# r-barnes/richdem

Hardware: NVIDIA H100
Metric: Priority-Flood fill + D8 flow accumulation throughput (higher is better)
Workload: dtype f32

## Files before the change

richdem_b200/csrc/capi.cu:

```cuda
#include "common.cuh"

#include <algorithm>
#include <cstdlib>

namespace rdb {

static thread_local std::string g_last_error;

void capi_set_error(const char *msg) { g_last_error = msg ? msg : "unknown error"; }

Ctx &ctx() {
  static Ctx c;
  return c;
}

static void init_device(int device) {
  Ctx &c = ctx();
  if (c.inited && c.device == device) return;
  if (c.inited) fail("rdb200_init: already initialised on device %d (call rdb200_shutdown first)", c.device);
  int ndev = 0;
  cudaError_t e = cudaGetDeviceCount(&ndev);
  if (e != cudaSuccess || ndev == 0)
    fail("no CUDA device available (%s); librichdem_b200 has no CPU fallback",
         e == cudaSuccess ? "device count is 0" : cudaGetErrorString(e));
// ... 136 lines not shown

}

using namespace rdb;

#define CAPI_TRY try {
#define CAPI_END                    \
  }                                 \
  catch (const std::exception &e) { \
    capi_set_error(e.what());       \
    return 1;                       \
  }                                 \
  catch (...) {                     \
    capi_set_error("unknown C++ exception"); \
    return 1;                       \
  }                                 \
  return 0;

extern "C" {

int rdb200_init(int device) {
  CAPI_TRY
  init_device(device);
  CAPI_END
}

void rdb200_shutdown(void) {
  Ctx &c = ctx();
  if (!c.inited) return;
  cudaSetDevice(c.device);
  cudaStreamSynchronize(c.stream);
  ws_release_all();
  if (c.pinned) cudaFreeHost(c.pinned);
  cudaEventDestroy(c.ev0);
  cudaEventDestroy(c.ev1);
  cudaEventDestroy(c.evk0);
  cudaEventDestroy(c.evk1);
  cudaStreamDestroy(c.own_stream);
  for (int k = 0; k < 2; k++)
    if (c.aux_stream[k]) cudaStreamDestroy(c.aux_stream[k]);
  for (int k = 0; k < 3; k++)
    if (c.aux_event[k]) cudaEventDestroy(c.aux_event[k]);
  const Params keep = c.params;
  c = Ctx();
  c.params = keep;
}

const char *rdb200_last_error(void) { return g_last_error.c_str(); }
int rdb200_version(void) { return RDB200_VERSION; }

int rdb200_set_stream(void *cuda_stream) {
  CAPI_TRY
  ensure_init();
  Ctx &c = ctx();
  RDB_CK(cudaStreamSynchronize(c.stream));
  c.stream = cuda_stream ? (cudaStream_t)cuda_stream : c.own_stream;
  CAPI_END
}

int rdb200_get_stats(rdb200_stats *out) {
  CAPI_TRY
  if (!out) fail("rdb200_get_stats: null pointer");
  *out = ctx().stats;
  CAPI_END
}

int rdb200_set_param(const char *name, int64_t value) {
  CAPI_TRY
  if (!name) fail("rdb200_set_param: null name");
  Params &p = ctx().params;
  const std::string n(name);
  if (n == "reset_defaults") p = Params();
  else if (n == "trim_workspace") {
    if (ctx().inited) {
      RDB_CK(cudaStreamSynchronize(ctx().stream));
      ws_trim();
    }
  }
  else if (n == "fill_max_iters") p.fill_max_iters = value;
  else if (n == "fill_rounds_per_sync") p.fill_rounds_per_sync = value > 0 ? value : 16;
  else if (n == "fill_use_tma") p.fill_use_tma = value;
  else if (n == "fill_external_z") p.fill_external_z = value;
  else if (n == "fill_profile") p.fill_profile = value;
  else if (n == "fill_trace") p.fill_trace = value;
  else if (n == "fill_ordered") p.fill_ordered = value;
  else if (n == "fill_order_rounds") p.fill_order_rounds = value;
  else if (n == "fill_band_rounds") p.fill_band_rounds = value;
  else if (n == "accum_threads") p.accum_threads = value > 0 ? value : 256;
  else if (n == "accum_budget") p.accum_budget = value;
  else if (n == "accum_walk_lanes") p.accum_walk_lanes = value;
  else if (n == "accum_fused_prep") p.accum_fused_prep = value;
  else if (n == "flats_tiled") p.flats_tiled = value;
  else if (n == "flats_pair") p.flats_pair = value;
  else if (n == "flats_fused_classify") p.flats_fused_classify = value;
  else if (n == "fill_multigrid") p.fill_multigrid = value;
  else if (n == "fill_multigrid_min") p.fill_multigrid_min = value;
  else if (n == "fill_vcycle") p.fill_vcycle = value;
  else if (n == "fill_band_multigrid") p.fill_band_multigrid = value;
  else if (n == "flats_uf_tiled") p.flats_uf_tiled = value;
  else if (n == "flowdirs_rolling") p.flowdirs_rolling = value;
  else if (n == "accum_packed") p.accum_packed = value;
  else if (n == "accum_dinf_packed") p.accum_dinf_packed = value;
  else if (n == "accum_dinf_share") p.accum_dinf_share = value;
  else if (n == "flowmet_tarboton_filter") p.flowmet_tarboton_filter = value;
  else if (n == "accum_walk_scan") p.accum_walk_scan = value;
  else if (n == "accum_walk_ahead") p.accum_walk_ahead = value;
  else if (n == "accum_dinf_stats") p.accum_dinf_stats = value;
  else if (n == "accum_dinf_wait") p.accum_dinf_wait = value;
  else fail("rdb200_set_param: unknown parameter '%s'", name);
  CAPI_END
}


int rdb200_fill_depressions_d8_f32(float *dem, int32_t w, int32_t h) {
  CAPI_TRY
  if (!dem) fail("fill_depressions: null dem");
  check_dims(w, h);
  CallScope cs((int64_t)w * h);
  const size_t n = (size_t)w * h;
  DevBuf<float> d(n);
  h2d(d.p, dem, n);
  fill_depressions_dev(d.p, w, h);
  d2h(dem, d.p, n);
  cs.done();
  CAPI_END
}

int rdb200_fill_depressions_d4_f32(float *dem, int32_t w, int32_t h) {
  CAPI_TRY
  if (!dem) fail("fill_depressions: null dem");
  check_dims(w, h);
  CallScope cs((int64_t)w * h);
  const size_t n = (size_t)w * h;
  DevBuf<float> d(n);
  h2d(d.p, dem, n);
  fill_depressions_dev(d.p, w, h, true);
  d2h(dem, d.p, n);
  cs.done();
  CAPI_END
}

static int pit_mask_host(const float *dem, uint8_t *mask, int32_t w, int32_t h, float nodata, bool topo4) {
  CAPI_TRY
  if (!dem || !mask) fail("pit_mask: null pointer");
  check_dims(w, h);
  CallScope cs((int64_t)w * h);
  const size_t n = (size_t)w * h;
  DevBuf<float> d(n);
  DevBuf<uint8_t> m(n);
  h2d(d.p, dem, n);
  pit_mask_dev(d.p, m.p, w, h, nodata, topo4);
  d2h(mask, m.p, n);
  cs.done();
  CAPI_END
}
int rdb200_pit_mask_d8_f32(const float *dem, uint8_t *mask, int32_t w, int32_t h, float nodata) {
  return pit_mask_host(dem, mask, w, h, nodata, false);
}
int rdb200_pit_mask_d4_f32(const float *dem, uint8_t *mask, int32_t w, int32_t h, float nodata) {
  return pit_mask_host(dem, mask, w, h, nodata, true);
}

static int has_depressions_host(const float *dem, int32_t w, int32_t h, int32_t *out, bool topo4) {
  CAPI_TRY
  if (!dem || !out) fail("has_depressions: null pointer");
  check_dims(w, h);
// ... 707 lines not shown
```

richdem_b200/csrc/common.cuh:

```cuda
#pragma once

#include <cuda.h>
#include <cuda_runtime.h>

#include <cstdarg>
#include <cstdint>
#include <cstdio>
#include <cstring>
#include <stdexcept>
#include <string>
#include <vector>

#include "../../include/richdem_b200.h"

struct rdb200_fill_state;

namespace rdb {

struct Error : std::runtime_error {
  using std::runtime_error::runtime_error;
};

[[noreturn]] inline void fail(const char *fmt, ...) {
  char buf[1024];
  va_list ap;
  va_start(ap, fmt);
  vsnprintf(buf, sizeof(buf), fmt, ap);
  va_end(ap);
  throw Error(buf);
}

#define RDB_CK(expr)                                                                        \
  do {                                                                                      \
    cudaError_t _e = (expr);                                                                \
    if (_e != cudaSuccess)                                                                  \
      ::rdb::fail("%s failed at %s:%d: %s", #expr, __FILE__, __LINE__, cudaGetErrorString(_e)); \
  } while (0)

__host__ __device__ __forceinline__ int d8dx(int n) {
  return (int)((0x6a41u >> (2 * n)) & 3u) - 1;
}
__host__ __device__ __forceinline__ int d8dy(int n) {
  return (int)((0x2a405u >> (2 * n)) & 3u) - 1;
}

struct Params {
  int64_t fill_max_iters = 0;
  int64_t fill_rounds_per_sync = 16;
  int64_t fill_use_tma = 1;
  int64_t fill_external_z = 1;
  int64_t fill_ordered = 1;
  int64_t fill_order_rounds = 0;
  int64_t fill_band_rounds = 0;
  int64_t fill_profile = 0;
  int64_t fill_trace = 0;
  int64_t fill_multigrid = 8;
  int64_t fill_vcycle = 8;
  int64_t fill_band_multigrid = 0;
  int64_t fill_multigrid_min = 0;
  int64_t flowdirs_rolling = 1;
  int64_t flats_uf_tiled = 1;
  int64_t flats_fused_classify = 1;
  int64_t flats_pair = 1;
  int64_t flats_tiled = 1;
  int64_t accum_dinf_packed = 1;
  int64_t flowmet_tarboton_filter = 1;
  int64_t accum_walk_ahead = 0;
  int64_t accum_walk_scan = 0;
  int64_t accum_dinf_stats = 0;
  int64_t accum_dinf_share = -1;
  int64_t accum_dinf_wait = 0;
  int64_t accum_packed = 1;
  int64_t accum_fused_prep = 1;
  int64_t accum_walk_lanes = 1;
  int64_t accum_threads = 256;
  int64_t accum_budget = 0;
};

struct WsBlock {
  void *ptr;
  size_t bytes;
  bool in_use;
};

struct Ctx {
  bool inited = false;
  int device = -1;
  int num_sms = 0;
  cudaStream_t stream = nullptr;
  cudaStream_t own_stream = nullptr;
  cudaEvent_t ev0 = nullptr, ev1 = nullptr, evk0 = nullptr, evk1 = nullptr;
  cudaStream_t aux_stream[2] = {nullptr, nullptr};
  cudaEvent_t aux_event[3] = {nullptr, nullptr, nullptr};
  std::vector<WsBlock> ws;
  void *pinned = nullptr;
  size_t pinned_bytes = 0;
  rdb200_stats stats;
  Params params;
};

Ctx &ctx();
void ensure_init();
void *ws_alloc(size_t bytes);
void ws_free(void *p);
void ws_release_all();

template <class T>
struct DevBuf {
  T *p = nullptr;
  size_t n = 0;
  DevBuf() = default;
  explicit DevBuf(size_t count) { alloc(count); }
  void alloc(size_t count) {
    reset();
    n = count;
    p = (T *)ws_alloc((count ? count : 1) * sizeof(T));
  }
  void reset() {
    if (p) ws_free(p);
    p = nullptr;
    n = 0;
  }
  ~DevBuf() { reset(); }
  DevBuf(const DevBuf &) = delete;
  DevBuf &operator=(const DevBuf &) = delete;
  operator T *() const { return p; }
};

inline void count_launch(int64_t k = 1) { ctx().stats.kernel_launches += k; }

struct KernelTimer {
  bool active;
  explicit KernelTimer(bool on = true) : active(on) {
    if (active) RDB_CK(cudaEventRecord(ctx().evk0, ctx().stream));
  }
  void stop_async() {
    if (active) RDB_CK(cudaEventRecord(ctx().evk1, ctx().stream));
// ... 69 lines not shown
```

richdem_b200/csrc/fill.cu:

```cuda
#include "common.cuh"

#include <chrono>

namespace rdb {

namespace {

#ifndef RDB_TX
#define RDB_TX 64
#endif
#ifndef RDB_TY
#define RDB_TY 64
#endif
#ifndef RDB_FILL_THREADS
#define RDB_FILL_THREADS 128
#endif
#ifndef RDB_FILL_MIN_CTAS
#define RDB_FILL_MIN_CTAS 6
#endif
constexpr int TX = RDB_TX;
constexpr int TY = RDB_TY;
constexpr int BXN = TX / 4;
constexpr int BYN = TY / 4;
constexpr int PADL = 4;
constexpr int SP = TX + 2 * PADL;
constexpr int SROWS = TY + 2;
constexpr int FILL_THREADS = RDB_FILL_THREADS;
constexpr int FILL_MIN_CTAS = RDB_FILL_MIN_CTAS;
static_assert(BYN <= 16 && BXN * BYN <= 256 && TX % 4 == 0 && TY % 4 == 0, "tile shape");
constexpr uint32_t W_TILE_BYTES = SP * SROWS * 4;
constexpr uint32_t Z_TILE_BYTES = TX * TY * 4;

struct RoundCtl {
  int count;
  int take;
};

struct FillDev {
  RoundCtl ctl[3];
  RoundCtl proc[3];
  unsigned long long visits;
  unsigned long long iters;
  unsigned long long block_updates;
  unsigned long long warp_updates;
  unsigned long long idle_visits;
  unsigned long long iter_hist[8];
  int edge_changed;
  int zmin_ord, zmax_ord;
  unsigned long long deferred;
  unsigned long long live_rounds;
  float level, step, step_min, level_max;
  int target, ordered;
  int ndefer[3];
};

struct FillArgs {
  const float *Z;
  int zpitch, zox, zoy;
  int inplace;
  const float *coarse;
  int Wc, pool, yoff;
  int *staged;
  float *zcopy;
  float *Wp;
  int pitch;
  int wox, woy;
  int W, H;
  int tilesX, tilesY;
  int *list0, *list1;
  int *stamp;
  int *sides;
  int *keys;
  float level;
  int *plist;
  int use_proc;
  FillDev *dev;
  int round;
  int max_iters;
  int use_tma;
  int profile;
  int *dirty;
};

__device__ __forceinline__ uint32_t smem_u32(const void *p) {
  return (uint32_t)__cvta_generic_to_shared(p);
}
__device__ __forceinline__ void mbar_init(unsigned long long *bar, int count) {
  asm volatile("mbarrier.init.shared::cta.b64 [%0], %1;" ::"r"(smem_u32(bar)), "r"(count) : "memory");
}
__device__ __forceinline__ void mbar_arrive_expect_tx(unsigned long long *bar, uint32_t bytes) {
  asm volatile("mbarrier.arrive.expect_tx.shared::cta.b64 _, [%0], %1;" ::"r"(smem_u32(bar)),
               "r"(bytes)
               : "memory");
}
__device__ __forceinline__ void mbar_wait(unsigned long long *bar, uint32_t parity) {
  uint32_t ok;
  const uint32_t addr = smem_u32(bar);
  do {
    asm volatile(
        "{\n"
        "  .reg .pred p;\n"
        "  mbarrier.try_wait.parity.shared::cta.b64 p, [%1], %2;\n"
        "  selp.u32 %0, 1, 0, p;\n"
        "}\n"
        : "=r"(ok)
        : "r"(addr), "r"(parity)
        : "memory");
  } while (!ok);
}
__device__ __forceinline__ void tma_load_2d(void *smem_dst, const CUtensorMap *map, int c0, int c1,
                                            unsigned long long *bar) {
  asm volatile(
      "cp.async.bulk.tensor.2d.shared::cluster.global.mbarrier::complete_tx::bytes [%0], [%1, {%2, %3}], [%4];"
      ::"r"(smem_u32(smem_dst)),
      "l"((unsigned long long)map), "r"(c0), "r"(c1), "r"(smem_u32(bar))
      : "memory");
}
__device__ __forceinline__ void fence_proxy_async() {
  asm volatile("fence.proxy.async.shared::cta;" ::: "memory");
}
__device__ __forceinline__ void tma_store_2d(const CUtensorMap *map, int c0, int c1, const void *smem_src) {
  asm volatile("cp.async.bulk.tensor.2d.global.shared::cta.bulk_group [%0, {%1, %2}], [%3];" ::"l"((unsigned long long)map),
               "r"(c0), "r"(c1), "r"(smem_u32(smem_src))
               : "memory");
  asm volatile("cp.async.bulk.commit_group;" ::: "memory");
}
__device__ __forceinline__ void bulk_wait_read() { asm volatile("cp.async.bulk.wait_group.read 0;" ::: "memory"); }
__device__ __forceinline__ void bulk_wait_all() { asm volatile("cp.async.bulk.wait_group 0;" ::: "memory"); }

constexpr int NBLK = BXN * BYN;
constexpr int MKP = BXN + 2;
constexpr int NWARP = FILL_THREADS / 32;
constexpr int SEG = ((NBLK + NWARP - 1) / NWARP + 31) / 32 * 32;
enum : int { SIDE_N = 1, SIDE_S = 2, SIDE_W = 4, SIDE_E = 8, SIDE_NW = 16, SIDE_NE = 32, SIDE_SW = 64,
             SIDE_SE = 128, SIDE_FULL = 256 };

__host__ __device__ __forceinline__ int f2ord(float f) {
  int b;
  memcpy(&b, &f, 4);
  return b >= 0 ? b : (b ^ 0x7fffffff);
}
__host__ __device__ __forceinline__ float ord2f(int o) {
  const int b = o >= 0 ? o : (o ^ 0x7fffffff);
  float f;
  memcpy(&f, &b, 4);
  return f;
}
constexpr int ORD_POS_INF = 0x7f800000;

__device__ __forceinline__ void enqueue_tile(const FillArgs &a, RoundCtl *next, int *list_next, int t,
                                             int stampval, int side_bits, int key_ord) {
  atomicOr(&a.sides[(stampval & 1) * a.tilesX * a.tilesY + t], side_bits);
  atomicMin(&a.keys[(stampval & 1) * a.tilesX * a.tilesY + t], key_ord);
  if (atomicExch(&a.stamp[t], stampval) != stampval) {
    const int idx = atomicAdd(&next->count, 1);
    list_next[idx] = t;
  }
}

__device__ __forceinline__ float min3f(float a, float b, float c) { return fminf(fminf(a, b), c); }

constexpr bool DRAIN_SWEEPS = TX == 64 && TY == 64 && FILL_THREADS == 128;

template <bool TOPO4>
__device__ __forceinline__ void fill_drain_sweeps(float *sW, const float *sZ, int y0, int H, int *sFlags, int *sKey) {
  const unsigned FULL = 0xffffffffu;
  const int tid = threadIdx.x, lane = tid & 31, wrp = tid >> 5;
  const int x = 32 * (wrp & 1) + lane;
  const bool down = wrp < 2;
  const int dy = down ? 1 : -1;
  const bool ecol = x < 4 || x >= TX - 4;
  unsigned long long rows = 0;
  float kmin = __int_as_float(0x7f800000);
  int y = down ? 0 : TY - 1;
  float p = sW[(y - dy + 1) * SP + PADL + x];
#pragma unroll 1
  for (int half = 0; half < 2; half++) {
#pragma unroll 8
    for (int s = 0; s < TY / 2; s++, y += dy) {
      const float zz = sZ[y * TX + x];
      float *cell = &sW[(y + 1) * SP + PADL + x];
      const float w = *cell;
      float m = p;
      if (!TOPO4) {
        float pl = __shfl_up_sync(FULL, p, 1), pr = __shfl_down_sync(FULL, p, 1);
        const float *prow = &sW[(y - dy + 1) * SP + PADL + x];
        if (lane == 0) pl = prow[-1];
        if (lane == 31) pr = prow[1];
        m = min3f(pl, p, pr);
      }
      const float nw = fminf(w, fmaxf(zz, m));
      p = w;
      if (nw < w) {
        *cell = nw;
        p = nw;
        rows |= 1ull << y;
        if (ecol || y < 4 || y >= TY - 4) kmin = fminf(kmin, nw);
      }
    }
    __syncthreads();
  }
  int f = 0;
#pragma unroll
  for (int by = 0; by < BYN; by++)
    if ((rows >> (4 * by)) & 0xFull) f |= 1 << (12 + by);
  if (rows & 1ull) f |= SIDE_N;
  if (rows >> (TY - 1)) f |= SIDE_S;
  if (x == 0 && rows) f |= SIDE_W | (rows & 1ull ? SIDE_NW : 0) | (rows >> (TY - 1) ? SIDE_SW : 0);
  if (x == TX - 1 && rows) f |= SIDE_E | (rows & 1ull ? SIDE_NE : 0) | (rows >> (TY - 1) ? SIDE_SE : 0);
  const int j1 = 1 - y0, j2 = (H - 2) - y0;
  if (j1 >= 0 && j1 < TY && ((rows >> j1) & 1ull)) f |= 1 << 9;
  if (j2 >= 0 && j2 < TY && ((rows >> j2) & 1ull)) f |= 1 << 10;
#pragma unroll
  for (int o = 16; o > 0; o >>= 1) {
    f |= __shfl_xor_sync(FULL, f, o);
    kmin = fminf(kmin, __shfl_xor_sync(FULL, kmin, o));
  }
  if (lane == 0 && f) {
    atomicOr(sFlags, f);
    if (f & 0xFF) atomicMin(sKey, f2ord(kmin));
  }
}

template <int STEP, bool TOPO4 = false, bool STAGE = false>
__global__ void __launch_bounds__(FILL_THREADS, FILL_MIN_CTAS)
    fill_sweep_kernel(const __grid_constant__ CUtensorMap mapW, const __grid_constant__ CUtensorMap mapZ,
                      const __grid_constant__ CUtensorMap mapZout, const FillArgs a) {
  __shared__ __align__(128) float sW[SROWS * SP];
  __shared__ __align__(128) float sZ[TY * TX];
  __shared__ __align__(8) unsigned long long mbar;
  __shared__ unsigned char sMark[MKP * (BYN + 2)];
  __shared__ unsigned char sList[2][NWARP][SEG];
  __shared__ __align__(16) int sCnt[2][NWARP];
  __shared__ int sTile;
  __shared__ int sFlags;
  __shared__ int sKey;
  __shared__ int sProf[2];
  __shared__ int sNbDone;

  const int tid = threadIdx.x;
  const int r = a.round;
  RoundCtl *cur = &a.dev->ctl[r % 3];
  RoundCtl *next = &a.dev->ctl[(r + 1) % 3];
  const int *list_cur = (r & 1) ? a.list1 : a.list0;
  int *list_next = (r & 1) ? a.list0 : a.list1;
  const int ntiles = a.tilesX * a.tilesY;
  if (a.use_proc) {
    cur = &a.dev->proc[r % 3];
    list_cur = a.plist;
  }
  const int n = cur->count;

  if (blockIdx.x == 0 && tid == 0) {
    RoundCtl *z = &a.dev->ctl[(r + 2) % 3];
    z->count = 0;
    z->take = 0;
    RoundCtl *zp = &a.dev->proc[(r + 1) % 3];
    zp->count = 0;
    zp->take = 0;
    if (n > 0) {
      atomicAdd(&a.dev->visits, (unsigned long long)n);
      a.dev->live_rounds++;
    }
  }
  if (n == 0) return;

  if (tid == 0) {
    mbar_init(&mbar, 1);
    asm volatile("fence.mbarrier_init.release.cluster;" ::: "memory");
  }
  uint32_t phase = 0;
  const int max_iters = a.max_iters;

  for (;;) {
    if (tid == 0) sTile = atomicAdd(&cur->take, 1);
    for (int k = tid; k < MKP * (BYN + 2); k += FILL_THREADS) sMark[k] = 0;
    __syncthreads();
    const int li = sTile;
    if (li >= n) break;
    const int t = list_cur[li];
    const int tyT = t / a.tilesX, txT = t - tyT * a.tilesX;
    const int x0 = txT * TX, y0 = tyT * TY;

    constexpr bool stage = STAGE;
    if (tid == 0) {
      sFlags = 0;
      sKey = ORD_POS_INF;
      sProf[0] = sProf[1] = 0;
      if (stage) {
        int nb = 0;
        for (int dy = -1; dy <= 1; dy++)
          for (int dx = -1; dx <= 1; dx++) {
            const int ty = tyT + dy, tx = txT + dx;
            if ((dx | dy) && ty >= 0 && ty < a.tilesY && tx >= 0 && tx < a.tilesX &&
                *reinterpret_cast<volatile int *>(&a.staged[ty * a.tilesX + tx]))
              nb |= 1 << ((dy + 1) * 3 + dx + 1);
          }
        __threadfence();
        sNbDone = nb;
      }
    }
    if (a.use_tma) {
      if (tid == 0) {
        fence_proxy_async();
        if (STAGE) bulk_wait_read();
        mbar_arrive_expect_tx(&mbar, (stage ? 0u : W_TILE_BYTES) + Z_TILE_BYTES);
        if (!stage) tma_load_2d(sW, &mapW, x0 - PADL + a.wox, y0 - 1 + a.woy, &mbar);
        tma_load_2d(sZ, &mapZ, x0 + a.zox, y0 + a.zoy, &mbar);
      }
    } else {
// ... 23 lines not shown
      a.keys[(r & 1) * ntiles + t] = ORD_POS_INF;
    }
    if (stage) {
      const float inf = __int_as_float(0x7f800000);
      const int nbdone = sNbDone;
      constexpr int C4N = SP / 4, RSTEP = FILL_THREADS / C4N;
      static_assert(RSTEP >= 1, "a CTA covers one row of the window");
      if (tid < RSTEP * C4N) {
        const int c4 = 4 * (tid % C4N);
        int rr = tid / C4N;
        const int dx = c4 < PADL ? -1 : (c4 >= PADL + TX ? 1 : 0);
        const int xb = x0 + c4 - PADL;
        const int cx = xb >= 0 ? xb / a.pool : 0, rx = xb - cx * a.pool;
        const int yy = y0 + rr - 1 + a.yoff;
        int cy = (yy + a.pool) / a.pool - 1, ry = yy - cy * a.pool;
        const int dq = RSTEP / a.pool, dr = RSTEP - dq * a.pool;
        for (; rr < SROWS; rr += RSTEP) {
          const int dy = rr == 0 ? -1 : (rr == SROWS - 1 ? 1 : 0);
          float4 v4;
          if (((nbdone >> ((dy + 1) * 3 + dx + 1)) & 1) && y0 + rr - 1 < a.H && xb < a.W) {
            v4 = __ldcg(reinterpret_cast<const float4 *>(a.Wp + (size_t)(y0 + rr - 1 + a.woy) * a.pitch + xb + a.wox));
          } else {
            const int y = y0 + rr - 1;
            float v[4] = {inf, inf, inf, inf};
            if (y >= 0 && y < a.H) {
              const float *crow = a.coarse + (size_t)cy * a.Wc;
              const float *zrow = a.Z + (size_t)(y + a.zoy) * a.zpitch + a.zox;
              const bool brow = y == 0 || y == a.H - 1;
              const float c0 = (a.pool & 3) == 0 && xb >= 0 && xb < a.W ? __ldg(crow + cx) : inf;
              int cc = cx, rc = rx;
#pragma unroll
              for (int j = 0; j < 4; j++) {
                const int x = xb + j;
                if (j > 0 && ++rc == a.pool) {
                  rc = 0;
                  cc++;
                }
                if (x >= 0 && x < a.W)
                  v[j] = brow || x == 0 || x == a.W - 1 ? __ldcg(zrow + x) : (a.pool & 3) == 0 ? c0 : __ldg(crow + cc);
              }
            }
            v4 = make_float4(v[0], v[1], v[2], v[3]);
          }
          *reinterpret_cast<float4 *>(&sW[rr * SP + c4]) = v4;
          cy += dq;
          ry += dr;
          if (ry >= a.pool) {
            ry -= a.pool;
            cy++;
          }
        }
      }
    }
#include "fill_relax_body.inc"

    if (f) {
      atomicOr(&sFlags, f);
      if (f & 0xFF) atomicMin(&sKey, f2ord(kmin));
    }
    __syncthreads();
    const int fl = sFlags;
    const int rowch = (fl >> 12) & 0xFFFF;
    const int rowout = stage ? (1 << BYN) - 1 : rowch;
    if (rowout) {
      for (int k = tid; k < TY * (TX / 4); k += FILL_THREADS) {
        const int rr = k / (TX / 4), cc = k % (TX / 4);
        const int y = y0 + rr, x = x0 + 4 * cc;
        if ((rowout & (1 << (rr >> 2))) && !(a.inplace && (y >= a.H || x >= a.W))) {
          const float4 val = *reinterpret_cast<const float4 *>(&sW[(rr + 1) * SP + PADL + 4 * cc]);
          __stcg(reinterpret_cast<float4 *>(a.Wp + (size_t)(y + a.woy) * a.pitch + x + a.wox), val);
          if (STAGE && !a.use_tma)
            __stcg(reinterpret_cast<float4 *>(a.zcopy + (size_t)y * a.W + x),
                   *reinterpret_cast<const float4 *>(&sZ[rr * TX + 4 * cc]));
        }
      }
    }
    if (stage) {
      __syncthreads();
      if (tid == 0) {
        __threadfence();
        atomicExch(&a.staged[t], 1);
      }
    }
    if (rowch) {
      if (tid < 8) {
        const int sv = r + 1;
        const bool n_ok = tyT > 0, s_ok = tyT < a.tilesY - 1, w_ok = txT > 0, e_ok = txT < a.tilesX - 1;
        int nb = -1, bits = 0;
        switch (tid) {
          case 0: if ((fl & SIDE_N) && n_ok) { nb = t - a.tilesX; bits = SIDE_S; } break;
          case 1: if ((fl & SIDE_S) && s_ok) { nb = t + a.tilesX; bits = SIDE_N; } break;
          case 2: if ((fl & SIDE_W) && w_ok) { nb = t - 1; bits = SIDE_E; } break;
          case 3: if ((fl & SIDE_E) && e_ok) { nb = t + 1; bits = SIDE_W; } break;
          case 4: if ((fl & SIDE_NW) && n_ok && w_ok) { nb = t - a.tilesX - 1; bits = SIDE_SE; } break;
          case 5: if ((fl & SIDE_NE) && n_ok && e_ok) { nb = t - a.tilesX + 1; bits = SIDE_SW; } break;
          case 6: if ((fl & SIDE_SW) && s_ok && w_ok) { nb = t + a.tilesX - 1; bits = SIDE_NE; } break;
          default: if ((fl & SIDE_SE) && s_ok && e_ok) { nb = t + a.tilesX + 1; bits = SIDE_NW; } break;
        }
        if (nb >= 0) enqueue_tile(a, next, list_next, nb, sv, bits, sKey);
        if (tid == 0 && (fl & (3 << 9))) atomicOr(&a.dev->edge_changed, (fl >> 9) & 3);
        if (tid == 0 && a.dirty) a.dirty[t] = 1;
      }
    }
    if (tid == 0) {
      if (again) enqueue_tile(a, next, list_next, t, r + 1, SIDE_FULL, f2ord(-__int_as_float(0x7f800000)));
      atomicAdd(&a.dev->iters, (unsigned long long)iters);
      if (a.profile) {
        if (!rowch) atomicAdd(&a.dev->idle_visits, 1ull);
        atomicAdd(&a.dev->block_updates, (unsigned long long)sProf[0]);
        atomicAdd(&a.dev->warp_updates, (unsigned long long)sProf[1]);
        const int hb = iters <= 1 ? 0 : iters <= 2 ? 1 : iters <= 4 ? 2 : iters <= 8 ? 3 : iters <= 16 ? 4 : iters <= 32 ? 5 : iters <= 64 ? 6 : 7;
        atomicAdd(&a.dev->iter_hist[hb], 1ull);
      }
    }
  }
  if (STAGE && a.use_tma && tid == 0) bulk_wait_all();
}

__global__ void __launch_bounds__(256) fill_admit_kernel(const FillArgs a) {
  const int r = a.round;
  const RoundCtl *cur = &a.dev->ctl[r % 3];
  RoundCtl *next = &a.dev->ctl[(r + 1) % 3];
  RoundCtl *proc = &a.dev->proc[r % 3];
  const int *list_cur = (r & 1) ? a.list1 : a.list0;
  int *list_next = (r & 1) ? a.list0 : a.list1;
  const int n = cur->count;
  const int ntiles = a.tilesX * a.tilesY;
  const float level = a.level;
  int nd = 0;
  for (int i = blockIdx.x * blockDim.x + threadIdx.x; i < n; i += gridDim.x * blockDim.x) {
    const int t = list_cur[i];
    const int kord = a.keys[(r & 1) * ntiles + t];
    if (ord2f(kord) <= level) {
      a.plist[atomicAdd(&proc->count, 1)] = t;
    } else {
      int bits = a.sides[(r & 1) * ntiles + t];
      if (bits == 0) bits = SIDE_FULL;
      a.sides[(r & 1) * ntiles + t] = 0;
      a.keys[(r & 1) * ntiles + t] = ORD_POS_INF;
      enqueue_tile(a, next, list_next, t, r + 1, bits, kord);
      nd++;
    }
  }
  for (int o = 16; o > 0; o >>= 1) nd += __shfl_xor_sync(0xffffffffu, nd, o);
  if ((threadIdx.x & 31) == 0 && nd) atomicAdd(&a.dev->ndefer[r % 3], nd);
}

__global__ void __launch_bounds__(256) fill_seed_kernel(const FillArgs a, const int *__restrict__ tiles, int n) {
  const int i = blockIdx.x * blockDim.x + threadIdx.x;
  if (i >= n) return;
  const int r = a.round;
  RoundCtl *cur = &a.dev->ctl[r % 3];
  int *list_cur = (r & 1) ? a.list1 : a.list0;
  enqueue_tile(a, cur, list_cur, tiles[i], r, SIDE_FULL, f2ord(-__int_as_float(0x7f800000)));
}

__global__ void __launch_bounds__(256) fill_seed_flags_kernel(const FillArgs a, const int *__restrict__ flag, int ntiles,
                                                               int *count) {
  const int t = blockIdx.x * blockDim.x + threadIdx.x;
  if (t >= ntiles || !flag[t]) return;
  const int r = a.round;
  RoundCtl *cur = &a.dev->ctl[r % 3];
  int *list_cur = (r & 1) ? a.list1 : a.list0;
  enqueue_tile(a, cur, list_cur, t, r, SIDE_FULL, f2ord(-__int_as_float(0x7f800000)));
  if (count) atomicAdd(count, 1);
}

// ... 271 lines not shown
        wv[j] = l;
        any = true;
        lo_w |= lx == 0;
        lo_e |= lx == TX - 1;
      }
    }
    if (any) {
      *wp4 = make_float4(wv[0], wv[1], wv[2], wv[3]);
      lowered = true;
      lo_n |= ly == 0;
      lo_s |= ly == TY - 1;
    }
  }
  if (lowered) {
    const int tilesY = (H + TY - 1) / TY;
    tile_flag[t] = 1;
    const bool n_ok = tyT > 0, s_ok = tyT < tilesY - 1, w_ok = txT > 0, e_ok = txT < tilesX - 1;
    if (lo_n && n_ok) tile_flag[t - tilesX] = 1;
    if (lo_s && s_ok) tile_flag[t + tilesX] = 1;
    if (lo_w && w_ok) tile_flag[t - 1] = 1;
    if (lo_e && e_ok) tile_flag[t + 1] = 1;
    if (lo_n && lo_w && n_ok && w_ok) tile_flag[t - tilesX - 1] = 1;
    if (lo_n && lo_e && n_ok && e_ok) tile_flag[t - tilesX + 1] = 1;
    if (lo_s && lo_w && s_ok && w_ok) tile_flag[t + tilesX - 1] = 1;
    if (lo_s && lo_e && s_ok && e_ok) tile_flag[t + tilesX + 1] = 1;
  }
}

__global__ void __launch_bounds__(256) fill_finish_x4_kernel(const float *__restrict__ Wp, float *__restrict__ out, int W,
                                                              int H, int pitch, int wox, int woy) {
  const int x4 = (blockIdx.x * blockDim.x + threadIdx.x) * 4;
  if (x4 >= W) return;
  for (int y = blockIdx.y; y < H; y += gridDim.y) {
    const float4 v = __ldcs(reinterpret_cast<const float4 *>(Wp + (size_t)(y + woy) * pitch + x4 + wox));
    __stcs(reinterpret_cast<float4 *>(out + (size_t)y * W + x4), v);
  }
}

__global__ void fill_finish_kernel(const float *__restrict__ Wp, float *__restrict__ out, int W, int H,
                                   int pitch, int wox, int woy) {
  const int x = blockIdx.x * blockDim.x + threadIdx.x;
  if (x >= W) return;
  for (int y = blockIdx.y; y < H; y += gridDim.y) out[(size_t)y * W + x] = Wp[(size_t)(y + woy) * pitch + x + wox];
}

typedef CUresult (*EncodeTiledFn)(CUtensorMap *, CUtensorMapDataType, cuuint32_t, void *, const cuuint64_t *,
                                  const cuuint64_t *, const cuuint32_t *, const cuuint32_t *,
                                  CUtensorMapInterleave, CUtensorMapSwizzle, CUtensorMapL2promotion,
                                  CUtensorMapFloatOOBfill);

EncodeTiledFn get_encode_fn() {
  static EncodeTiledFn fn = nullptr;
  if (!fn) {
    void *p = nullptr;
    cudaDriverEntryPointQueryResult q;
    RDB_CK(cudaGetDriverEntryPoint("cuTensorMapEncodeTiled", &p, cudaEnableDefault, &q));
    if (!p || q != cudaDriverEntryPointSuccess) fail("cuTensorMapEncodeTiled not available from the driver");
    fn = (EncodeTiledFn)p;
  }
  return fn;
}

CUtensorMap make_map(float *base, int pitch, int rows, int boxw, int boxh) {
  CUtensorMap m;
  const cuuint64_t gdim[2] = {(cuuint64_t)pitch, (cuuint64_t)rows};
  const cuuint64_t gstride[1] = {(cuuint64_t)pitch * 4};
  const cuuint32_t box[2] = {(cuuint32_t)boxw, (cuuint32_t)boxh};
  const cuuint32_t estr[2] = {1, 1};
  CUresult rc = get_encode_fn()(&m, CU_TENSOR_MAP_DATA_TYPE_FLOAT32, 2, base, gdim, gstride, box, estr,
                                CU_TENSOR_MAP_INTERLEAVE_NONE, CU_TENSOR_MAP_SWIZZLE_NONE,
                                CU_TENSOR_MAP_L2_PROMOTION_L2_128B, CU_TENSOR_MAP_FLOAT_OOB_FILL_NONE);
  if (rc != CUDA_SUCCESS) fail("cuTensorMapEncodeTiled failed with CUresult %d", (int)rc);
  return m;
}

}

struct FillState {
  int W = 0, H = 0, pitch = 0, rows = 0, tilesX = 0, tilesY = 0;
  DevBuf<float> Zp, Wp;
  DevBuf<int> list0, list1, plist, stamp, sides, keys;
  DevBuf<int> dirty, tflag;
  DevBuf<int> staged;
  float zmin = 0.f, zmax = 0.f;
  bool first_run = true;
  bool ordered = false;
  int step_mode = 0;
  bool topo4 = false;
  std::vector<float> levels;
  DevBuf<FillDev> dev;
  CUtensorMap mapW, mapZ;
  int round = 0;
  int grid = 0;
  int64_t rounds_run = 0;
  int64_t live_rounds = 0;
  int64_t visits_seen = 0;
  bool still_active = false;
  int64_t sched_round = 0;

  float *Wb = nullptr;
  int wpitch = 0, wox = 0, woy = 0;
  bool inplace = false;
  DevBuf<float> Zc;
  const float *stage_coarse = nullptr;
  int stage_wc = 0, stage_k = 1, stage_yoff = 0;
  CUtensorMap mapZstage;

  void use_padded_layout(size_t np) {
    inplace = false;
    Zc.reset();
    Zp.alloc(np);
    Wp.alloc(np);
    Wb = Wp.p;
    wpitch = pitch;
    wox = PADL;
    woy = 1;
  }

  void begin(const float *d_dem, int w, int h, const float *d_coarse = nullptr, int coarse_w = 0, int coarse_k = 0,
             int coarse_yoff = 0, bool in_place = false) {
    Ctx &c = ctx();
    W = w;
    H = h;
    tilesX = (w + TX - 1) / TX;
    tilesY = (h + TY - 1) / TY;
    pitch = tilesX * TX + 2 * PADL;
    rows = tilesY * TY + 2;
    const size_t np = (size_t)pitch * rows;
    if (in_place && c.params.fill_external_z != 0 && (w & 3) == 0 && ((uintptr_t)d_dem & 15) == 0) {
      inplace = true;
      Zp.reset();
      Wp.reset();
      Zc.alloc((size_t)w * h);
      Wb = const_cast<float *>(d_dem);
      wpitch = w;
      wox = woy = 0;
    } else {
      use_padded_layout(np);
    }
    stage_coarse = inplace && d_coarse ? d_coarse : nullptr;
    stage_wc = coarse_w;
    stage_k = coarse_k;
    stage_yoff = coarse_yoff;
    const size_t nt = (size_t)tilesX * tilesY;
    list0.alloc(nt);
    list1.alloc(nt);
    plist.alloc(nt);
    stamp.alloc(nt);
    sides.alloc(2 * nt);
    keys.alloc(2 * nt);
    dev.alloc(1);
    RDB_CK(cudaMemsetAsync(stamp.p, 0, nt * sizeof(int), c.stream));
    RDB_CK(cudaMemsetAsync(sides.p, 0, 2 * nt * sizeof(int), c.stream));
    if (stage_coarse) {
      staged.alloc(nt);
      RDB_CK(cudaMemsetAsync(staged.p, 0, nt * sizeof(int), c.stream));
    }
    {
      FillDev h0;
      memset(&h0, 0, sizeof(h0));
      h0.zmin_ord = ORD_POS_INF;
      h0.zmax_ord = f2ord(-__builtin_inff());
      memcpy(c.pinned, &h0, sizeof(h0));
      RDB_CK(cudaMemcpyAsync(dev.p, c.pinned, sizeof(FillDev), cudaMemcpyHostToDevice, c.stream));
    }
    {
      const int n2 = (int)(2 * nt);
      fill_i32_kernel<<<(n2 + 255) / 256, 256, 0, c.stream>>>(keys.p, ORD_POS_INF, n2);
      count_launch();
      dim3 blk(128), grd((pitch / 4 + 127) / 128, rows < 2048 ? rows : 2048);
      if (stage_coarse) {
      } else if (inplace) {
        dim3 grdc((W / 4 + 127) / 128, H < 2048 ? H : 2048);
        fill_init_kernel<false><<<grdc, blk, 0, c.stream>>>(d_dem, Zc.p, Wb, W, H, W, H, 0, 0, dev.p, nullptr, 0, 1, 0);
        count_launch();
      } else if (d_coarse) {
        fill_init_kernel<true><<<grd, blk, 0, c.stream>>>(d_dem, Zp.p, Wp.p, W, H, pitch, rows, PADL, 1, dev.p, d_coarse,
                                                         coarse_w, coarse_k, coarse_yoff);
        count_launch();
      } else {
        fill_init_kernel<false><<<grd, blk, 0, c.stream>>>(d_dem, Zp.p, Wp.p, W, H, pitch, rows, PADL, 1, dev.p, nullptr, 0, 1,
                                                          0);
        count_launch();
      }
      RDB_CK(cudaGetLastError());
      zmin = zmax = 0.f;
      if (!d_coarse) {
        FillDev *hd = (FillDev *)c.pinned;
        RDB_CK(cudaMemcpyAsync(hd, dev.p, sizeof(FillDev), cudaMemcpyDeviceToHost, c.stream));
        RDB_CK(cudaStreamSynchronize(c.stream));
        zmin = ord2f(hd->zmin_ord);
        zmax = ord2f(hd->zmax_ord);
        if (!(zmin <= zmax)) zmin = zmax = 0.f;
      }
      ordered = c.params.fill_ordered != 0 && zmax > zmin && !d_coarse;
      levels.clear();
      if (ordered) {
        int64_t R = c.params.fill_order_rounds;
        if (R <= 0) R = (int64_t)(0.8 * (tilesX > tilesY ? tilesX : tilesY));
        if (R < 8) {
          ordered = false;
        } else {
          DevBuf<unsigned int> hist(HIST_BINS);
          RDB_CK(cudaMemsetAsync(hist.p, 0, HIST_BINS * sizeof(unsigned int), c.stream));
          const int stride = rows > 4096 ? 16 : (rows > 512 ? 4 : 1);
          const int nb = (rows - 2 + stride - 1) / stride;
          if (inplace)
            fill_hist_kernel<<<nb, 256, 0, c.stream>>>(Zc.p, W, W, H, stride, zmin, 1.0f / (zmax - zmin), hist.p);
          else
            fill_hist_kernel<<<nb, 256, 0, c.stream>>>(Zp.p + pitch, pitch, pitch, rows - 1, stride, zmin, 1.0f / (zmax - zmin),
                                                       hist.p);
          RDB_CK(cudaGetLastError());
          count_launch();
          unsigned int *hh = (unsigned int *)c.pinned;
          RDB_CK(cudaMemcpyAsync(hh, hist.p, HIST_BINS * sizeof(unsigned int), cudaMemcpyDeviceToHost, c.stream));
          RDB_CK(cudaStreamSynchronize(c.stream));
          double total = 0;
          for (int k = 0; k < HIST_BINS; k++) total += hh[k];
          levels.resize((size_t)R);
          double cum = 0;
          int bin = 0;
          for (int64_t k = 0; k < R; k++) {
            const double want = total * (double)(k + 1) / (double)R;
            while (bin < HIST_BINS - 1 && cum + hh[bin] < want) cum += hh[bin++];
            levels[(size_t)k] = zmin + (zmax - zmin) * (float)(bin + 1) / (float)HIST_BINS;
          }
        }
      }
    }
    if (inplace) {
      mapW = make_map(Wb, W, H, SP, SROWS);
      mapZ = make_map(Zc.p, W, H, TX, TY);
      if (stage_coarse) mapZstage = make_map(Wb, W, H, TX, TY);
    } else {
      mapW = make_map(Wp.p, pitch, rows, SP, SROWS);
      mapZ = make_map(Zp.p, pitch, rows, TX, TY);
    }
    int per_sm = 0;
    RDB_CK(cudaOccupancyMaxActiveBlocksPerMultiprocessor(&per_sm, fill_sweep_kernel<0>, FILL_THREADS, 0));
    if (per_sm < 1) per_sm = 1;
// ... 18 lines not shown
    rows = tilesY * TY + 2;
    use_padded_layout((size_t)pitch * rows);
    const size_t nt = (size_t)tilesX * tilesY;
    list0.alloc(nt);
    list1.alloc(nt);
    plist.alloc(nt);
    stamp.alloc(nt);
    sides.alloc(2 * nt);
    keys.alloc(2 * nt);
    dev.alloc(1);
    RDB_CK(cudaMemsetAsync(stamp.p, 0, nt * sizeof(int), c.stream));
    RDB_CK(cudaMemsetAsync(sides.p, 0, 2 * nt * sizeof(int), c.stream));
    RDB_CK(cudaMemsetAsync(dev.p, 0, sizeof(FillDev), c.stream));
    const int n2 = (int)(2 * nt);
    fill_i32_kernel<<<(n2 + 255) / 256, 256, 0, c.stream>>>(keys.p, ORD_POS_INF, n2);
    dim3 blk(128), grd((pitch + 127) / 128, rows < 2048 ? rows : 2048);
    clear_flags();
    dist_pad_init_kernel<<<grd, blk, 0, c.stream>>>(d_open, open_bit, d_winit, Zp.p, Wp.p, W, H, pitch, rows, ghost_top,
                                                    ghost_bottom, tflag.p, tilesX);
    RDB_CK(cudaGetLastError());
    count_launch(2);
    ordered = false;
    mapW = make_map(Wp.p, pitch, rows, SP, SROWS);
    mapZ = make_map(Zp.p, pitch, rows, TX, TY);
    int per_sm = 0;
    RDB_CK(cudaOccupancyMaxActiveBlocksPerMultiprocessor(&per_sm, fill_sweep_kernel<1>, FILL_THREADS, 0));
    if (per_sm < 1) per_sm = 1;
    grid = c.num_sms * per_sm;
    round = 1;
    seed_from_flags();
  }

  void seed_worklist(const std::vector<int> &tiles) {
    Ctx &c = ctx();
    if (tiles.empty()) return;
    DevBuf<int> d(tiles.size());
    RDB_CK(cudaMemcpyAsync(d.p, tiles.data(), tiles.size() * sizeof(int), cudaMemcpyHostToDevice, c.stream));
    FillArgs a = make_args();
    a.round = round;
    fill_seed_kernel<<<(unsigned)((tiles.size() + 255) / 256), 256, 0, c.stream>>>(a, d.p, (int)tiles.size());
    RDB_CK(cudaGetLastError());
    count_launch();
    RDB_CK(cudaStreamSynchronize(c.stream));
  }

  FillArgs make_args() {
    Ctx &c = ctx();
    FillArgs a;
    memset(&a, 0, sizeof(a));
    if (inplace) {
      a.Z = Zc.p;
      a.zpitch = W;
      a.inplace = 1;
    } else {
      a.Z = Zp.p;
      a.zpitch = pitch;
      a.zox = PADL;
      a.zoy = 1;
    }
    a.Wc = stage_wc;
    a.pool = stage_k;
    a.yoff = stage_yoff;
    a.staged = staged.p;
    a.Wp = Wb;
    a.pitch = wpitch;
    a.wox = wox;
    a.woy = woy;
    a.W = W;
    a.H = H;
    a.tilesX = tilesX;
    a.tilesY = tilesY;
    a.list0 = list0.p;
    a.list1 = list1.p;
    a.stamp = stamp.p;
    a.sides = sides.p;
    a.keys = keys.p;
    a.plist = plist.p;
    a.dev = dev.p;
    a.max_iters = (int)c.params.fill_max_iters;
    a.use_tma = (int)c.params.fill_use_tma;
    a.profile = (int)c.params.fill_profile;
    a.level = __builtin_inff();
    a.dirty = dirty.p;
    return a;
  }

  bool timed = true;
  int batch_edge = 0;
  void launch_batch(int per_sync) {
    Ctx &c = ctx();
    FillArgs a = make_args();
    if (timed) RDB_CK(cudaEventRecord(c.evk0, c.stream));
    for (int k = 0; k < per_sync; k++) {
      a.round = round;
      if (ordered && sched_round < (int64_t)levels.size()) {
        a.level = levels[(size_t)sched_round];
        a.use_proc = 1;
        fill_admit_kernel<<<c.num_sms * 2, 256, 0, c.stream>>>(a);
        c.stats.kernel_launches++;
      } else {
        a.level = __builtin_inff();
        a.use_proc = 0;
      }
      sched_round++;
      a.coarse = round == 1 ? stage_coarse : nullptr;
      a.Z = a.coarse ? Wb : (inplace ? Zc.p : Zp.p);
      a.zcopy = a.coarse ? Zc.p : nullptr;
      const CUtensorMap &mz = a.coarse ? mapZstage : mapZ;
      if (step_mode) fill_sweep_kernel<1><<<grid, FILL_THREADS, 0, c.stream>>>(mapW, mz, mapZ, a);
      else if (a.coarse && topo4) fill_sweep_kernel<0, true, true><<<grid, FILL_THREADS, 0, c.stream>>>(mapW, mz, mapZ, a);
      else if (a.coarse) fill_sweep_kernel<0, false, true><<<grid, FILL_THREADS, 0, c.stream>>>(mapW, mz, mapZ, a);
      else if (topo4) fill_sweep_kernel<0, true><<<grid, FILL_THREADS, 0, c.stream>>>(mapW, mz, mapZ, a);
      else fill_sweep_kernel<0><<<grid, FILL_THREADS, 0, c.stream>>>(mapW, mz, mapZ, a);
      round++;
    }
    if (timed) RDB_CK(cudaEventRecord(c.evk1, c.stream));
    RDB_CK(cudaGetLastError());
    RDB_CK(cudaMemcpyAsync(c.pinned, dev.p, sizeof(FillDev), cudaMemcpyDeviceToHost, c.stream));
    c.stats.kernel_launches += per_sync;
    rounds_run += per_sync;
    if (round > (1 << 30)) fail("fill: round counter overflow");
  }
  bool collect() {
    Ctx &c = ctx();
    RDB_CK(cudaStreamSynchronize(c.stream));
    if (timed) {
      float t = 0;
      RDB_CK(cudaEventElapsedTime(&t, c.evk0, c.evk1));
      c.stats.ms_main_kernel += t;
    }
    const FillDev *hd = (const FillDev *)c.pinned;
    still_active = hd->ctl[round % 3].count != 0;
    if (!still_active) first_run = false;
    live_rounds = (int64_t)hd->live_rounds;
    visits_seen = (int64_t)hd->visits;
    iters_seen = (int64_t)hd->iters;
    batch_edge = hd->edge_changed;
    return still_active;
  }
  int64_t iters_seen = 0;

  int run(int64_t max_rounds = 0) {
    Ctx &c = ctx();
    int64_t rounds_this_call = 0;
    int per_sync = (int)(c.params.fill_rounds_per_sync > 0 ? c.params.fill_rounds_per_sync : 16);
    if (max_rounds > 0 && max_rounds < per_sync) per_sync = (int)max_rounds;
    RDB_CK(cudaMemsetAsync(&dev.p->edge_changed, 0, sizeof(int), c.stream));
    for (;;) {
      launch_batch(per_sync);
      collect();
      rounds_this_call += per_sync;
      if (!still_active) break;
      if (max_rounds > 0 && rounds_this_call >= max_rounds) break;
    }
    const FillDev *hd = (const FillDev *)c.pinned;
    c.stats.fill_rounds = live_rounds;
    c.stats.fill_tile_visits = visits_seen;
    c.stats.fill_tile_iters = iters_seen;
    c.stats.fill_tile_cells = TX * TY;
    if (c.params.fill_profile) {
      fprintf(stderr, "[fill profile] deferred=%llu visits=%llu iters=%llu block_updates=%llu (%.1f%% of 256/iter) warp_updates=%llu (%.1f%% of 8/iter) idle_visits=%llu hist(1,2,3-4,5-8,9-16,17-32,33-64,65+)=",
              hd->deferred, hd->visits, hd->iters, hd->block_updates, 100.0 * hd->block_updates / (256.0 * hd->iters + 1),
              hd->warp_updates, 100.0 * hd->warp_updates / (8.0 * hd->iters + 1), hd->idle_visits);
      for (int k = 0; k < 8; k++) fprintf(stderr, "%llu ", hd->iter_hist[k]);
      fprintf(stderr, "\n");
    }
    return batch_edge | (still_active ? 4 : 0);
  }

  void track_dirty() {
    Ctx &c = ctx();
    const size_t nt = (size_t)tilesX * tilesY;
    dirty.alloc(nt);
    RDB_CK(cudaMemsetAsync(dirty.p, 0, nt * sizeof(int), c.stream));
  }
  void clear_dirty() {
    if (dirty.p) RDB_CK(cudaMemsetAsync(dirty.p, 0, (size_t)tilesX * tilesY * sizeof(int), ctx().stream));
  }
  void seed_from_flags(int *d_count = nullptr) {
    Ctx &c = ctx();
    const int nt = tilesX * tilesY;
    FillArgs a = make_args();
    a.round = round;
    fill_seed_flags_kernel<<<(nt + 255) / 256, 256, 0, c.stream>>>(a, tflag.p, nt, d_count);
    RDB_CK(cudaGetLastError());
    count_launch();
  }
  void clear_flags() {
    const size_t nt = (size_t)tilesX * tilesY;
    if (!tflag.p) tflag.alloc(nt);
    RDB_CK(cudaMemsetAsync(tflag.p, 0, nt * sizeof(int), ctx().stream));
  }
  void restrict_into(FillState &cs, int k) {
    Ctx &c = ctx();
    cs.clear_flags();
    const bool selective = dirty.p && TX % k == 0 && TY % k == 0;
    dim3 blk(256), grd((unsigned)((cs.W + 255) / 256), (unsigned)(cs.H < 4096 ? cs.H : 4096));
    fill_restrict_kernel<<<grd, blk, 0, c.stream>>>(Wb, wpitch, wox, woy, W, H, cs.Wb, cs.wpitch, cs.wox, cs.woy, cs.W, cs.H,
                                                    k, selective ? dirty.p : nullptr, tilesX, cs.tflag.p, cs.tilesX);
    RDB_CK(cudaGetLastError());
    count_launch();
    cs.seed_from_flags();
    clear_dirty();
  }
  void blockmax_into(float *d_out, int wc, int hc, int k, int yoff, int y_lo, int y_hi, bool selective = false) {
    Ctx &c = ctx();
    dim3 blk(256), grd((unsigned)((wc + 255) / 256), (unsigned)((y_hi - y_lo) / k + 2 < 4096 ? (y_hi - y_lo) / k + 2 : 4096));
    const bool sel = selective && dirty.p && TX % k == 0;
    fill_blockmax_kernel<<<grd, blk, 0, c.stream>>>(Wb, wpitch, wox, woy, W, y_lo, y_hi, yoff, d_out, wc, hc, k,
                                                    sel ? dirty.p : nullptr, tilesX);
    RDB_CK(cudaGetLastError());
    count_launch();
    if (sel) clear_dirty();
  }
  void prolong_from(const float *d_wc, int cpitch, int coff_x, int coff_y, int k, int yoff = 0, const int *cdirty = nullptr,
                    int ctilesX = 0, int *d_count = nullptr) {
    Ctx &c = ctx();
    clear_flags();
    const int nt = tilesX * tilesY;
    fill_prolong_kernel<<<nt, 256, 0, c.stream>>>(Wb, wpitch, wox, woy, W, H, d_wc, cpitch, coff_x, coff_y, k, tflag.p, tilesX,
                                                  yoff, cdirty, ctilesX);
    RDB_CK(cudaGetLastError());
    count_launch();
    seed_from_flags(d_count);
  }
  void prolong_from_level(FillState &cs, int k, int yoff = 0, int *d_count = nullptr) {
    prolong_from(cs.Wb, cs.wpitch, cs.wox, cs.woy, k, yoff, cs.dirty.p, cs.tilesX, d_count);
    cs.clear_dirty();
  }
  void ghost_update(int y, const float *d_row, int *d_lowered) {
    Ctx &c = ctx();
    clear_flags();
    fill_ghost_update_kernel<<<(W + 255) / 256, 256, 0, c.stream>>>(Wp.p, Zp.p, pitch, W, H, y, d_row, tflag.p, tilesX, d_lowered);
    RDB_CK(cudaGetLastError());
    count_launch();
    seed_from_flags();
  }

  void read_row(int y, float *d_row) {
    if (y < 0 || y >= H) fail("fill_read_row: row %d out of range", y);
    RDB_CK(cudaMemcpyAsync(d_row, Wb + (size_t)(y + woy) * wpitch + wox, (size_t)W * 4,
                           cudaMemcpyDeviceToDevice, ctx().stream));
  }

  void update_row(int y, const float *d_row) {
    if (y != 0 && y != H - 1) fail("fill_update_row: only boundary rows (0, height-1) can be replaced");
    Ctx &c = ctx();
    const size_t o = (size_t)(y + 1) * pitch + PADL;
    RDB_CK(cudaMemcpyAsync(Wp.p + o, d_row, (size_t)W * 4, cudaMemcpyDeviceToDevice, c.stream));
    RDB_CK(cudaMemcpyAsync(Zp.p + o, d_row, (size_t)W * 4, cudaMemcpyDeviceToDevice, c.stream));
    pending_rows.push_back(y);
// ... 569 lines not shown
```

Baseline: 21580.

## Filter tile wake-ups using per-edge above-water bitmasks

```diff
diff --git a/richdem_b200/csrc/capi.cu b/richdem_b200/csrc/capi.cu
--- a/richdem_b200/csrc/capi.cu
+++ b/richdem_b200/csrc/capi.cu
@@ -242,6 +242,7 @@
   else if (n == "fill_use_tma") p.fill_use_tma = value;
   else if (n == "fill_external_z") p.fill_external_z = value;
   else if (n == "fill_profile") p.fill_profile = value;
+  else if (n == "fill_wake_filter") p.fill_wake_filter = value;
   else if (n == "fill_trace") p.fill_trace = value;
   else if (n == "fill_ordered") p.fill_ordered = value;
   else if (n == "fill_order_rounds") p.fill_order_rounds = value;
diff --git a/richdem_b200/csrc/common.cuh b/richdem_b200/csrc/common.cuh
--- a/richdem_b200/csrc/common.cuh
+++ b/richdem_b200/csrc/common.cuh
@@ -53,6 +53,7 @@
   int64_t fill_order_rounds = 0;
   int64_t fill_band_rounds = 0;
   int64_t fill_profile = 0;
+  int64_t fill_wake_filter = 1;
   int64_t fill_trace = 0;
   int64_t fill_multigrid = 8;
   int64_t fill_vcycle = 8;
diff --git a/richdem_b200/csrc/fill.cu b/richdem_b200/csrc/fill.cu
--- a/richdem_b200/csrc/fill.cu
+++ b/richdem_b200/csrc/fill.cu
@@ -44,6 +44,7 @@
   unsigned long long block_updates;
   unsigned long long warp_updates;
   unsigned long long idle_visits;
+  unsigned long long wakes_dropped;
   unsigned long long iter_hist[8];
   int edge_changed;
   int zmin_ord, zmax_ord;
@@ -80,6 +81,7 @@
   int use_tma;
   int profile;
   int *dirty;
+  unsigned long long *edge_above;
 };
 
 __device__ __forceinline__ uint32_t smem_u32(const void *p) {
@@ -159,6 +161,20 @@
 }
 
 __device__ __forceinline__ float min3f(float a, float b, float c) { return fminf(fminf(a, b), c); }
+
+constexpr bool WAKE_WORDS = TX <= 64 && TY <= 64;
+
+struct EdgeLine {
+  int len, o, st, da, zo, zs;
+};
+__device__ __forceinline__ EdgeLine edge_line(int s) {
+  switch (s) {
+    case 0: return {TX, SP + PADL, 1, -SP, 0, 1};
+    case 1: return {TX, TY * SP + PADL, 1, SP, (TY - 1) * TX, 1};
+    case 2: return {TY, SP + PADL, SP, -1, 0, TX};
+    default: return {TY, SP + PADL + TX - 1, SP, 1, TX - 1, TX};
+  }
+}
 
 constexpr bool DRAIN_SWEEPS = TX == 64 && TY == 64 && FILL_THREADS == 128;
 
@@ -222,10 +238,65 @@
   }
 }
 
+#ifndef __noinline__
+#define __noinline__ __attribute__((noinline))
+#endif
+template <bool TOPO4>
+__device__ __noinline__ void fill_wake_neighbours(const FillArgs &a, const float *sW, const float *sZ, int t, int fl, int key,
+                                                  RoundCtl *next, int *list_next) {
+  const unsigned FULL = 0xffffffffu;
+  const int lane = threadIdx.x & 31;
+  const int tyT = t / a.tilesX, txT = t - tyT * a.tilesX;
+  const bool n_ok = tyT > 0, s_ok = tyT < a.tilesY - 1, w_ok = txT > 0, e_ok = txT < a.tilesX - 1;
+  const int sv = a.round + 1;
+  for (int s = threadIdx.x >> 5; s < 4; s += NWARP) {
+    const EdgeLine e = edge_line(s);
+    unsigned long long word = 0;
+    for (int i0 = 0; i0 < e.len; i0 += 32) {
+      const int i = i0 + lane;
+      const bool above = i < e.len && !(sW[e.o + i * e.st] == sZ[e.zo + i * e.zs]);
+      word |= (unsigned long long)__ballot_sync(FULL, above) << i0;
+    }
+    if (lane == 0) __stcg(&a.edge_above[(size_t)t * 4 + s], word);
+    if (!((fl >> 12) & 0xFFFF)) continue;
+    if (!TOPO4 && lane == 1 && (fl & (SIDE_NW << s))) {
+      const bool north = s < 2, west = (s & 1) == 0;
+      if ((north ? n_ok : s_ok) && (west ? w_ok : e_ok)) {
+        const int nb = t + (north ? -a.tilesX : a.tilesX) + (west ? -1 : 1);
+        const int own = (north ? SP : TY * SP) + PADL + (west ? 0 : TX - 1);
+        const int across = own + (north ? -SP : SP) + (west ? -1 : 1);
+        const unsigned long long nword = __ldcg(&a.edge_above[(size_t)nb * 4 + (north ? 1 : 0)]);
+        if (((nword >> (west ? TX - 1 : 0)) & 1ull) && sW[own] < sW[across])
+          enqueue_tile(a, next, list_next, nb, sv, SIDE_NW << (3 - s), key);
+        else if (a.profile)
+          atomicAdd(&a.dev->wakes_dropped, 1ull);
+      }
+    }
+    if (!((fl >> s) & 1) || !(s == 0 ? n_ok : s == 1 ? s_ok : s == 2 ? w_ok : e_ok)) continue;
+    const int nb = s == 0 ? t - a.tilesX : s == 1 ? t + a.tilesX : s == 2 ? t - 1 : t + 1;
+    const unsigned long long nword = __ldcg(&a.edge_above[(size_t)nb * 4 + (s ^ 1)]);
+    bool need = false;
+    for (int i = lane; i < e.len; i += 32) {
+      if (!((nword >> i) & 1ull)) continue;
+      float m = sW[e.o + i * e.st];
+      if (!TOPO4) {
+        if (i > 0) m = fminf(m, sW[e.o + (i - 1) * e.st]);
+        if (i < e.len - 1) m = fminf(m, sW[e.o + (i + 1) * e.st]);
+      }
+      need |= m < sW[e.o + i * e.st + e.da];
+    }
+    if (__ballot_sync(FULL, need)) {
+      if (lane == 0) enqueue_tile(a, next, list_next, nb, sv, 1 << (s ^ 1), key);
+    } else if (lane == 0 && a.profile) {
+      atomicAdd(&a.dev->wakes_dropped, 1ull);
+    }
+  }
+}
+
 template <int STEP, bool TOPO4 = false, bool STAGE = false>
 __global__ void __launch_bounds__(FILL_THREADS, FILL_MIN_CTAS)
     fill_sweep_kernel(const __grid_constant__ CUtensorMap mapW, const __grid_constant__ CUtensorMap mapZ,
-                      const __grid_constant__ CUtensorMap mapZout, const FillArgs a) {
+                      const __grid_constant__ CUtensorMap mapZout, const __grid_constant__ FillArgs a) {
   __shared__ __align__(128) float sW[SROWS * SP];
   __shared__ __align__(128) float sZ[TY * TX];
   __shared__ __align__(8) unsigned long long mbar;
@@ -415,7 +486,13 @@
         atomicExch(&a.staged[t], 1);
       }
     }
-    if (rowch) {
+    if (STEP == 0 && WAKE_WORDS && a.edge_above) {
+      fill_wake_neighbours<TOPO4>(a, sW, sZ, t, fl, sKey, next, list_next);
+      if (rowch && tid == 0) {
+        if (fl & (3 << 9)) atomicOr(&a.dev->edge_changed, (fl >> 9) & 3);
+        if (a.dirty) a.dirty[t] = 1;
+      }
+    } else if (rowch) {
       if (tid < 8) {
         const int sv = r + 1;
         const bool n_ok = tyT > 0, s_ok = tyT < a.tilesY - 1, w_ok = txT > 0, e_ok = txT < a.tilesX - 1;
@@ -853,6 +930,7 @@
   DevBuf<int> list0, list1, plist, stamp, sides, keys;
   DevBuf<int> dirty, tflag;
   DevBuf<int> staged;
+  DevBuf<unsigned long long> edge_above;
   float zmin = 0.f, zmax = 0.f;
   bool first_run = true;
   bool ordered = false;
@@ -927,6 +1005,8 @@
       staged.alloc(nt);
       RDB_CK(cudaMemsetAsync(staged.p, 0, nt * sizeof(int), c.stream));
     }
+    edge_above.alloc(4 * nt);
+    RDB_CK(cudaMemsetAsync(edge_above.p, 0xff, 4 * nt * sizeof(unsigned long long), c.stream));
     {
       FillDev h0;
       memset(&h0, 0, sizeof(h0));
@@ -1111,6 +1191,7 @@
     a.profile = (int)c.params.fill_profile;
     a.level = __builtin_inff();
     a.dirty = dirty.p;
+    a.edge_above = step_mode == 0 && c.params.fill_wake_filter != 0 ? edge_above.p : nullptr;
     return a;
   }
 
@@ -1188,14 +1269,20 @@
     c.stats.fill_tile_iters = iters_seen;
     c.stats.fill_tile_cells = TX * TY;
     if (c.params.fill_profile) {
-      fprintf(stderr, "[fill profile] deferred=%llu visits=%llu iters=%llu block_updates=%llu (%.1f%% of 256/iter) warp_updates=%llu (%.1f%% of 8/iter) idle_visits=%llu hist(1,2,3-4,5-8,9-16,17-32,33-64,65+)=",
+      fprintf(stderr, "[fill profile] deferred=%llu visits=%llu iters=%llu block_updates=%llu (%.1f%% of 256/iter) warp_updates=%llu (%.1f%% of 8/iter) idle_visits=%llu wakes_dropped=%llu hist(1,2,3-4,5-8,9-16,17-32,33-64,65+)=",
               hd->deferred, hd->visits, hd->iters, hd->block_updates, 100.0 * hd->block_updates / (256.0 * hd->iters + 1),
-              hd->warp_updates, 100.0 * hd->warp_updates / (8.0 * hd->iters + 1), hd->idle_visits);
+              hd->warp_updates, 100.0 * hd->warp_updates / (8.0 * hd->iters + 1), hd->idle_visits, hd->wakes_dropped);
       for (int k = 0; k < 8; k++) fprintf(stderr, "%llu ", hd->iter_hist[k]);
       fprintf(stderr, "\n");
+      fprintf(stderr, "[fill wake] visits=%llu idle_visits=%llu wakes_dropped=%llu\n", hd->visits - prof_seen[0],
+              hd->idle_visits - prof_seen[1], hd->wakes_dropped - prof_seen[2]);
+      prof_seen[0] = hd->visits;
+      prof_seen[1] = hd->idle_visits;
+      prof_seen[2] = hd->wakes_dropped;
     }
     return batch_edge | (still_active ? 4 : 0);
   }
+  unsigned long long prof_seen[3] = {0, 0, 0};
 
   void track_dirty() {
     Ctx &c = ctx();
```

After: 22380, median of 6. 1.04x the previous value.
